# applied-geodesy/bundle-adjustment

Measured on AMD Instinct MI355X. Metric: LM iterations/sec, higher is better.
Workload: dtype f64

## Files before the change

### bundle-adjustment_amd/csrc/cholflow.hip

```cpp
#include <hip/hip_runtime.h>
#include <stdio.h>
#include <stdlib.h>
#include <string.h>

#include <algorithm>
#include <chrono>
#include <mutex>
#include <thread>
#include <vector>

#include "dense.h"
#include "gemm_f64.h"
#include "potrf_diag.h"

namespace jaicov {

#define HIPCHK(x)                                  \
    do {                                           \
        hipError_t _e = (x);                       \
        if (_e != hipSuccess) return _e;           \
    } while (0)

enum { FLOW_TICKET = 0, FLOW_ABORT = 1, FLOW_DIAG_NEXT = 2, FLOW_CHAIN_AT = 3, FLOW_STALE = 4, FLOW_STALE_CONFIRMED = 5, FLOW_RESCUED = 6, FLOW_WG_OFF = 7, FLOW_CTRL_WORDS = 16 };
constexpr int FLOW_FIN = 1 << 20;
constexpr int FLOW_PART = 1 << 21;
constexpr int FLOW_NPART_SHIFT = 22;
constexpr int FLOW_BUF_SHIFT = 12;
constexpr int FLOW_LDS = 144;
constexpr int FLOW_STAGE = GEMM_BK * 2 * FLOW_LDS;

struct FlowArgs {
    double *L;
    long ld;
    double *invd;
    const int4 *tasks;
    int n_tasks;
    int nb;
    int fs;
    int *ctrl;
    int *done;
    int *applied;
    int *diag_ready;
    int *factored;
    int *info;
    int *alive;
    int seq;
    const double *src;
    long src_ld;
    const double *V;
    const double *Bh;
    int d, U, bstride;
    double *diag_scratch;
    const double *zeros;
    double *scratch;
    double *partial;
    int *pflag;
    long long timeout;
    int fake_a;
    int crit_prio;
    int keep;
    int second_wg;
    int second_update;
    int inv_wt;
    int crit_span;
    int *wgstate;
    long long *ctrace;
    long long *trace;
};

__device__ __forceinline__ int flow_ld(const int *p) { return __hip_atomic_load(p, __ATOMIC_RELAXED, __HIP_MEMORY_SCOPE_AGENT); }
__device__ __forceinline__ int flow_ld_rmw(const int *p) { return __hip_atomic_fetch_or(const_cast<int *>(p), 0, __ATOMIC_RELAXED, __HIP_MEMORY_SCOPE_AGENT); }
__device__ __forceinline__ void flow_st(int *p, int v) { __hip_atomic_store(p, v, __ATOMIC_RELAXED, __HIP_MEMORY_SCOPE_SYSTEM); }
__device__ __forceinline__ int flow_ld_sys(const int *p) { return __hip_atomic_load(p, __ATOMIC_RELAXED, __HIP_MEMORY_SCOPE_SYSTEM); }
__device__ __forceinline__ void store_wt(double *p, double v) {
    __hip_atomic_store(reinterpret_cast<unsigned long long *>(p), (unsigned long long)__double_as_longlong(v), __ATOMIC_RELAXED,
                       __HIP_MEMORY_SCOPE_AGENT);
}
__device__ __forceinline__ void store_wt2(double *p, d2_t v) {
    asm volatile("s_nop 15\n\ts_nop 7\n\tglobal_store_dwordx4 %0, %1, off sc1\n\ts_nop 1" : : "v"(p), "v"(v) : "memory");
}
__device__ __forceinline__ void drain_stores() { asm volatile("s_waitcnt vmcnt(0)" ::: "memory"); }
#ifndef FLOW_LONG_NAP
#define FLOW_LONG_NAP 40
#endif

#define FLOW_OPAQUE_TID(name) int name = tid; asm volatile("" : "+v"(name))

__device__ __forceinline__ void flow_give_up(int *ctrl) {
    if (atomicCAS(ctrl + FLOW_ABORT, 0, 2) == 0) {
        int *wg = ctrl + ctrl[FLOW_WG_OFF];
        for (int b = 0; b < 1024; b++) wg[1024 + b] = flow_ld(wg + b);
    }
}

__device__ __forceinline__ bool flow_spin(const int *flag, int want, int *ctrl, long long timeout, long long *waited) {
    if (flow_ld(flag) >= want) return true;
    const long long t0 = wall_clock64();
    int spins = 0;
    bool ok = true;
    for (;;) {
        if (flow_ld(flag) >= want) break;
        if (++spins < 32) __builtin_amdgcn_s_sleep(4);
        else {
            __builtin_amdgcn_s_sleep(FLOW_LONG_NAP);
            if ((spins & 31) == 0) {
                if (flow_ld_sys(flag) >= want || flow_ld_rmw(flag) >= want) {
                    atomicAdd(ctrl + FLOW_STALE, 1);
                    if (flow_ld(flag) < want) atomicAdd(ctrl + FLOW_STALE_CONFIRMED, 1);
                    if (wall_clock64() - t0 > 100000) atomicAdd(ctrl + FLOW_RESCUED, 1);
                    break;
                }
                if (flow_ld(ctrl + FLOW_ABORT) != 0) { ok = false; break; }
                if (wall_clock64() - t0 > timeout) { flow_give_up(ctrl); ok = false; break; }
            }
        }
    }
    if (waited) *waited += wall_clock64() - t0;
    return ok;
}

__device__ __attribute__((noinline)) void flow_inline_diag(double *A, long ld, double *inv_out, int *info, int blk, double *ws) {
    potrf_diag_body(A, ld, inv_out, info, blk, 0, ws, ws + 128 * DP);
}

template <int PF, bool INLINE_DIAG>
__global__ __launch_bounds__(256, 2) void chol_tile_kernel(FlowArgs g) {
    __shared__ double smem[2 * FLOW_STAGE];
    __shared__ int s_msg[4];
    const int tid = threadIdx.x;
    const int bid = (int)blockIdx.x;

    d4_t acc[4][4];
    auto accumulate = [&](const double *Ap, long lda, const double *Bp, long ldb, int nk, double asign) __attribute__((always_inline)) {
        FLOW_OPAQUE_TID(tq);
        const int seg = tq & 7, rbase = tq >> 3, lane = tq & 63, wave = tq >> 6;
        const int odd = (seg & 1) * FLOW_LDS;
        const int st_lds = (2 * seg) * FLOW_LDS + rbase + 8 * ((seg >> 1) & 1) + 4 * (seg >> 2);
        const int fa = (lane >> 4) * FLOW_LDS + 64 * (wave >> 1) + (lane & 15);
        const int fb = (lane >> 4) * FLOW_LDS + 64 * (wave & 1) + (lane & 15);
        const double *ap = Ap + (long)rbase * lda + 2 * seg;
        const double *bp = Bp + (long)rbase * ldb + 2 * seg;
        d2_t ra[2][4], rb[2][4];
#define FLOW_GLOAD(S)                                                                                        \
    do {                                                                                                     \
        _Pragma("unroll") for (int q = 0; q < 4; q++) ra[S][q] = *reinterpret_cast<const d2_t *>(ap + (long)(32 * q) * lda); \
        _Pragma("unroll") for (int q = 0; q < 4; q++) rb[S][q] = *reinterpret_cast<const d2_t *>(bp + (long)(32 * q) * ldb); \
        ++ls;                                                                                                \
        const long adv = ls < nk ? GEMM_BK : 0;    \
        ap += adv;                                                                                           \
        bp += adv;                                                                                           \
    } while (0)
#define FLOW_LSTORE(S, STAGE)                                                                                \
    do {                                                                                                     \
        double *sa = smem + (STAGE) * FLOW_STAGE + st_lds;                                                   \
        double *sb = sa + GEMM_BK * FLOW_LDS;                                                                \
        _Pragma("unroll") for (int q = 0; q < 4; q++) {                                                      \
            sa[32 * q + odd] = asign * ra[S][q].x;                                                           \
            sa[32 * q + FLOW_LDS - odd] = asign * ra[S][q].y;                                                \
            sb[32 * q + odd] = rb[S][q].x;                                                                   \
            sb[32 * q + FLOW_LDS - odd] = rb[S][q].y;                                                        \
        }                                                                                                    \
    } while (0)
#define FLOW_FRAG(STAGE, KS, A_, B_)                                                                         \
    do {                                                                                                     \
        const double *sa = smem + (STAGE) * FLOW_STAGE + fa;                                                 \
        const double *sb = smem + (STAGE) * FLOW_STAGE + GEMM_BK * FLOW_LDS + fb;                            \
        const int sh = 8 * ((KS) & 1) + 4 * ((KS) >> 1);                                                     \
        _Pragma("unroll") for (int x = 0; x < 4; x++) A_[x] = sa[(4 * (KS)) * FLOW_LDS + 16 * x + sh];       \
        _Pragma("unroll") for (int y = 0; y < 4; y++) B_[y] = sb[(4 * (KS)) * FLOW_LDS + 16 * y + sh];       \
    } while (0)
#define FLOW_MM(A_, B_)                                                                                      \
    do {                                                                                                     \
        _Pragma("unroll") for (int x = 0; x < 4; x++)                                                        \
            _Pragma("unroll") for (int y = 0; y < 4; y++)                                                    \
                acc[x][y] = __builtin_amdgcn_mfma_f64_16x16x4f64(A_[x], B_[y], acc[x][y], 0, 0, 0);          \
    } while (0)
#define FLOW_MFMA(STAGE)                                                                                     \
    do {                                                                                                     \
        _Pragma("unroll") for (int ks = 0; ks < 4; ks++) {                                                   \
            double a[4], b[4];                                                                               \
            FLOW_FRAG(STAGE, ks, a, b);                                                                      \
            FLOW_MM(a, b);                                                                                   \
        }                                                                                                    \
    } while (0)
        int ls = 0;
        FLOW_GLOAD(0);
        if (PF == 2) {
            FLOW_GLOAD(1);
            FLOW_LSTORE(0, 0);
            __syncthreads();
            for (int kt = 0; kt < nk; kt += 2) {
                FLOW_GLOAD(0);
                FLOW_MFMA(0);
                FLOW_LSTORE(1, 1);
                __syncthreads();
                FLOW_GLOAD(1);
                FLOW_MFMA(1);
                FLOW_LSTORE(0, 0);
                __syncthreads();
            }
        } else {
            FLOW_LSTORE(0, 0);
            __syncthreads();
            for (int kt = 0; kt < nk; kt += 2) {
                FLOW_GLOAD(0);
                FLOW_MFMA(0);
                FLOW_LSTORE(0, 1);
                __syncthreads();
                FLOW_GLOAD(0);
                FLOW_MFMA(1);
                FLOW_LSTORE(0, 0);
                __syncthreads();
            }
        }
#undef FLOW_GLOAD
#undef FLOW_LSTORE
#undef FLOW_MFMA
#undef FLOW_FRAG
#undef FLOW_MM
    };

    if (!INLINE_DIAG && g.keep > 0 && (int)blockIdx.x >= g.keep) {
        const int xcc = 1 + (int)(__builtin_amdgcn_s_getreg((20 << 0) | (0 << 6) | (31 << 11)) & 0xf);
        if (xcc == flow_ld(g.ctrl + 9) || xcc == flow_ld(g.ctrl + 11) || (g.second_wg && xcc == flow_ld(g.ctrl + 13))) return;
    }
    for (;;) {
        if (tid == 0) s_msg[0] = atomicAdd(g.ctrl + FLOW_TICKET, 1);
        __syncthreads();
        const int t = s_msg[0];
        __syncthreads();
        if (t >= g.n_tasks) break;
        const int4 tk = g.tasks[t];
        const int ti = tk.x, tj = tk.y, k0 = tk.z & ((1 << FLOW_BUF_SHIFT) - 1), k1 = tk.w & (FLOW_FIN - 1);
        const int pbuf = tk.z >> FLOW_BUF_SHIFT, npart = (tk.w >> FLOW_NPART_SHIFT) & 7;
        const bool part = (tk.w & FLOW_PART) != 0;
        const bool first_visit = k0 == 0 || npart > 0;
#define FLOW_STAGE_MARK(kk, st) do { if (tid == 0) flow_st(g.wgstate + bid, (t << 12) | ((kk) << 4) | (st)); } while (0)
        FLOW_STAGE_MARK(k0, 1);
        const bool fin = (tk.w & FLOW_FIN) != 0;
        long long waited = 0, t_start = 0, t_c = 0, t_upd = 0, c_c = 0, c_upd = 0, w_upd = 0;
        int n_runs = 0;
        if (g.trace) t_start = wall_clock64();
        bool ok = true;
        const bool critical = ti <= tj + g.crit_span && g.crit_prio > 0;
        if (critical) __builtin_amdgcn_s_setprio(3);
        int k = k0;
        for (int phase = 0;; phase++) {
            if ((phase == 0 && !first_visit && !part) || phase == 1) {
                FLOW_STAGE_MARK(k, 2);
                if (tid == 0) {
                    const int *f = phase == 0 ? g.applied + (long)ti * g.fs + tj : g.done + (long)tj * g.fs + tj;
                    const bool r = flow_spin(f, phase == 0 ? k0 + 1 : 1, g.ctrl, g.timeout, &waited);
                    __builtin_amdgcn_fence(__ATOMIC_ACQUIRE, "agent");
                    drain_stores();
                    s_msg[1] = r ? 1 : 0;
                }
                __syncthreads();
                ok = s_msg[1] != 0;
                __syncthreads();
                if (!ok) break;
            }
            {
                FLOW_OPAQUE_TID(tq);
                const long trow = 64 * (tq >> 7) + ((tq & 63) >> 4), tcol = 64 * ((tq >> 6) & 1) + (tq & 15);
                const bool scaled = phase == 0 && first_visit && !part && g.src != nullptr && ti < g.nb;
                const double *src = phase != 0 || part ? g.zeros + (tq & 15)
                                    : scaled   ? g.src + ((long)ti * 128 + trow) * g.src_ld + (long)tj * 128 + tcol
                                               : g.L + ((long)ti * 128 + trow) * g.ld + (long)tj * 128 + tcol;
                const long sld = phase != 0 || part ? 0 : (scaled ? g.src_ld : g.ld);
#pragma unroll
                for (int x = 0; x < 4; x++)
#pragma unroll
                    for (int r = 0; r < 4; r++) {
                        const double *rowp = src + (long)(16 * x + 4 * r) * sld;
#pragma unroll
                        for (int y = 0; y < 4; y++) acc[x][y][r] = rowp[16 * y];
                    }
                if (scaled) {
                    const int R0 = ti * 128 + (int)trow, C0 = tj * 128 + (int)tcol;
                    double vc[4];
#pragma unroll
                    for (int y = 0; y < 4; y++) vc[y] = g.V[C0 + 16 * y];
#pragma unroll
                    for (int x = 0; x < 4; x++)
#pragma unroll
                        for (int r = 0; r < 4; r++) {
                            const int R = R0 + 16 * x + 4 * r;
                            const double vr = g.V[R];
#pragma unroll
                            for (int y = 0; y < 4; y++) {
                                const int Cc = C0 + 16 * y;
                                double v = vr * acc[x][y][r] * vc[y];
                                for (int a = 0; a < g.d; a++) v += g.Bh[(long)a * g.bstride + R] * g.Bh[(long)a * g.bstride + Cc];
                                const bool inside = R >= g.d && R < g.U && Cc >= g.d;
                                acc[x][y][r] = inside ? v : (R == Cc ? 1.0 : 0.0);
                            }
                        }
                }
            }
            if (g.trace && phase == 0) { t_c = wall_clock64(); c_c = clock64(); }
            for (bool more = true; more;) {
                const double *Ap, *Bp;
                long lda, ldb;
                int nk;
                double asign;
                if (phase == 0) {
                    if (k >= k1) break;
                    FLOW_STAGE_MARK(k, 3);
                    if (tid < 64) {
                        FLOW_OPAQUE_TID(lane);
                        const int *fi = g.done + (long)ti * g.fs, *fj = g.done + (long)tj * g.fs;
                        const long long t0 = wall_clock64();
                        int spins = 0, cnt = 0;
                        for (;;) {
                            const int idx = k + lane;
                            const bool ready = idx < k1 && flow_ld(fi + idx) != 0 && flow_ld(fj + idx) != 0;
                            const unsigned long long m = __ballot(ready);
                            cnt = m == ~0ull ? 64 : __builtin_ctzll(~m);
                            if (cnt > 0) break;
                            if (++spins < 32) __builtin_amdgcn_s_sleep(4);
                            else {
                                __builtin_amdgcn_s_sleep(FLOW_LONG_NAP);
                                if ((spins & 31) == 0) {
                                    if (wall_clock64() - t0 > 100000) {
                                        __builtin_amdgcn_fence(__ATOMIC_ACQUIRE, "agent");
                                        drain_stores();
                                    }
                                    const bool ready2 = idx < k1 && (flow_ld_sys(fi + idx) != 0 || flow_ld_rmw(fi + idx) != 0) &&
                                                        (flow_ld_sys(fj + idx) != 0 || flow_ld_rmw(fj + idx) != 0);
                                    const unsigned long long m2 = __ballot(ready2);
                                    cnt = m2 == ~0ull ? 64 : __builtin_ctzll(~m2);
                                    if (cnt > 0) {
                                        const bool again = idx < k1 && flow_ld(fi + idx) != 0 && flow_ld(fj + idx) != 0;
                                        const unsigned long long m3 = __ballot(again);
                                        if (lane == 0) {
                                            atomicAdd(g.ctrl + FLOW_STALE, 1);
                                            if ((m3 & 1ull) == 0) atomicAdd(g.ctrl + FLOW_STALE_CONFIRMED, 1);
                                            if (wall_clock64() - t0 > 100000) atomicAdd(g.ctrl + FLOW_RESCUED, 1);
                                        }
                                        break;
                                    }
                                    if (flow_ld(g.ctrl + FLOW_ABORT) != 0) break;
                                    if (wall_clock64() - t0 > g.timeout) { if (lane == 0) flow_give_up(g.ctrl); break; }
                                }
                            }
                        }
                        if (spins > 0) waited += wall_clock64() - t0;
                        __builtin_amdgcn_fence(__ATOMIC_ACQUIRE, "agent");
                        drain_stores();
                        if (lane == 0) {
                            s_msg[1] = cnt;
                            s_msg[2] = spins;
                        }
                    }
                    __syncthreads();
                    const int cnt = s_msg[1];
                    if (g.crit_prio >= 2 && s_msg[2] > 0) __builtin_amdgcn_s_setprio(3);
                    __syncthreads();
                    if (cnt == 0) { ok = false; break; }
                    ++n_runs;
                    FLOW_STAGE_MARK(k, 4);
                    Ap = g.L + (long)(g.fake_a ? tj : ti) * 128 * g.ld + (long)k * 128;
                    Bp = g.L + (long)tj * 128 * g.ld + (long)k * 128;
                    lda = ldb = g.ld;
                    nk = 8 * cnt;
                    asign = -1.0;
                    k += cnt;
                } else {
                    Ap = g.scratch + (long)bid * 16384;
                    Bp = g.invd + (long)tj * 16384;
                    lda = ldb = 128;
                    nk = 8;
                    asign = 1.0;
                    more = false;
                }
                accumulate(Ap, lda, Bp, ldb, nk, asign);
            }
            if (!ok) break;
            if (phase == 0 && npart > 0) {
                for (int q = 0; q < npart; q++) {
                    FLOW_STAGE_MARK(k, 9);
                    if (tid == 0) {
                        const bool r = flow_spin(g.pflag + pbuf + q, 1, g.ctrl, g.timeout, &waited);
                        __builtin_amdgcn_fence(__ATOMIC_ACQUIRE, "agent");
                        drain_stores();
                        s_msg[1] = r ? 1 : 0;
                    }
                    __syncthreads();
                    ok = s_msg[1] != 0;
                    __syncthreads();
                    if (!ok) break;
                    FLOW_OPAQUE_TID(tq);
                    const double *pp = g.partial + (long)(pbuf + q) * 16384 + (64 * (tq >> 7) + ((tq & 63) >> 4)) * 128 + 64 * ((tq >> 6) & 1) + (tq & 15);
#pragma unroll
                    for (int x = 0; x < 4; x++)
#pragma unroll
                        for (int r = 0; r < 4; r++)
#pragma unroll
                            for (int y = 0; y < 4; y++) acc[x][y][r] += pp[(16 * x + 4 * r) * 128 + 16 * y];
                }
                if (!ok) break;
            }
            if (g.trace && phase == 0) { t_upd = wall_clock64(); c_upd = clock64(); w_upd = waited; }
            FLOW_STAGE_MARK(k, 5 + phase);
            const bool to_scratch = phase == 0 && fin && ti != tj;
            {
                FLOW_OPAQUE_TID(tq);
                const long trow = 64 * (tq >> 7) + ((tq & 63) >> 4), tcol = 64 * ((tq >> 6) & 1) + (tq & 15);
                double *dst = part         ? g.partial + (long)pbuf * 16384 + trow * 128 + tcol
                              : to_scratch ? g.scratch + (long)bid * 16384 + trow * 128 + tcol
                                           : g.L + ((long)ti * 128 + trow) * g.ld + (long)tj * 128 + tcol;
                const long dld = part || to_scratch ? 128 : g.ld;
#pragma unroll
                for (int x = 0; x < 4; x++)
#pragma unroll
                    for (int r = 0; r < 4; r++) {
                        double *rowp = dst + (long)(16 * x + 4 * r) * dld;
#pragma unroll
                        for (int y = 0; y < 4; y++) store_wt(rowp + 16 * y, acc[x][y][r]);
                    }
            }
            drain_stores();
            if (to_scratch) continue;
            __syncthreads();
            if (INLINE_DIAG && phase == 0 && fin) {
                if (tid == 0) {
                    __builtin_amdgcn_fence(__ATOMIC_ACQUIRE, "agent");
                    drain_stores();
                }
                __syncthreads();
                double *ws = g.diag_scratch + (long)bid * (128 * DP + 8 * 16 * WDP);
                flow_inline_diag(g.L + (long)tj * 128 * g.ld + (long)tj * 128, g.ld, g.invd + (long)tj * 16384, g.info, tj, ws);
                drain_stores();
                __syncthreads();
                if (tid == 0) {
                    __builtin_amdgcn_fence(__ATOMIC_RELEASE, "agent");
                    drain_stores();
                    flow_st(g.done + (long)tj * g.fs + tj, 1);
                }
                break;
            }
            if (tid == 0) {
                if (part) flow_st(g.pflag + pbuf, 1);
                else if (phase == 1) flow_st(g.done + (long)ti * g.fs + tj, 1);
                else if (fin) flow_st(g.diag_ready + tj, 1);
                else flow_st(g.applied + (long)ti * g.fs + tj, k1 + 1);
            }
            break;
        }
        if (g.crit_prio > 0) __builtin_amdgcn_s_setprio(0);
        FLOW_STAGE_MARK(k, ok ? 7 : 8);
        if (!ok) break;
        if (g.trace && tid == 0) {
            long long *tr = g.trace + 8 * (long)t;
            tr[0] = t_start; tr[1] = t_c; tr[2] = t_upd; tr[3] = wall_clock64(); tr[4] = waited;
            tr[5] = c_upd - c_c;
            tr[6] = (long long)bid | ((long long)n_runs << 16) | (w_upd << 32);
            tr[7] = (long long)__builtin_amdgcn_s_getreg((4 << 0) | (0 << 6) | (31 << 11)) |
                    ((long long)(__builtin_amdgcn_s_getreg((20 << 0) | (0 << 6) | (31 << 11)) & 0xf) << 32);
// ... 797 lines not shown
```

### bundle-adjustment_amd/csrc/engine.hip

```cpp
#include <hip/hip_runtime.h>
#include <math.h>
#include <stdio.h>
#include <string.h>

#include <algorithm>
#include <atomic>
#include <chrono>
#include <string>
#include <vector>

#include "../../include/jaicov_dense.h"
#include "../../include/jaicov_neq.h"
#include "ba_kernels.h"
#include "batchinv.h"
#include "datum.h"
#include "dense.h"
#include "gemm_f64.h"
#include "reliability.h"
#include "transform.h"

namespace jaicov {
hipError_t launch_rows(hipStream_t, const DevProblem &, const double *, int, int, double *, double *);
hipError_t launch_assemble_small(hipStream_t, const DevProblem &, const int32_t *, const int32_t *, int, const double *,
                                 const double *, double, double *, double *);
hipError_t launch_assemble_blocks(hipStream_t, const DevProblem &, const int32_t *, int, int, const int32_t *, int,
                                  const double *, const double *, double *, double, double *, double *, const PPGather &,
                                  const SchurBufs &, double *, hipStream_t, hipEvent_t, hipEvent_t);
hipError_t launch_schur_backsub(hipStream_t, const DevProblem &, const int32_t *, int, const double *, const double *,
                                const double *, double *);
hipError_t launch_shared_groups(hipStream_t, const DevProblem &, const double *, double, double *, double *,
                                const double *, double *);
hipError_t launch_schur_expand_f(hipStream_t, const DevProblem &, const int32_t *, int, const double *, const double *, const double *,
                                 const double *, double *, long);
hipError_t launch_omega(hipStream_t, const DevProblem &, const uint8_t *, int, int, const int32_t *, int, int,
                        const double *, const double *, const double *, double, double *, double *);
struct RefineBorder { double kappa[7]; double rk[7]; };
hipError_t launch_residual_dd(hipStream_t, const double *, long, int, int, int, const double *, const double *, const double *,
                              const double *, const double *, long, const RefineBorder &, double *, double *);
}
using namespace jaicov;

static const double EPS53 = 1.1102230246251565e-16;

__global__ void damp_and_precond_kernel(double *N, long ld, int U, int Upad, int d, double lambda, double *V,
                                        const double *diagcorr) {
    const int c = blockIdx.x * blockDim.x + threadIdx.x;
    if (c >= Upad) return;
    double v = 1.0;
    if (c >= d && c < U) {
        double diag = N[(long)c * ld + c];
        if (lambda > 0.0) {
            diag += lambda * (diag + (diagcorr ? diagcorr[c] : 0.0));
            N[(long)c * ld + c] = diag;
        }
        v = diag > 1.1102230246251565e-16 ? 1.0 / sqrt(diag) : 1.0;
    }
    V[c] = v;
}

__global__ __launch_bounds__(256) void zero_lower_kernel(double *__restrict__ N, long ld, int rows, int skip_lo, int skip_hi, int row0) {
    const int r = row0 + blockIdx.y, c = 4 * (blockIdx.x * 256 + threadIdx.x);
    if (c > r || r >= rows) return;
    if (r >= skip_lo && r <= skip_hi) {
        if (c >= skip_lo) return;
        if (c + 4 > skip_lo) {
            for (int k = c; k < skip_lo; k++) N[(long)r * ld + k] = 0.0;
            return;
        }
    }
    *reinterpret_cast<d4_t *>(N + (long)r * ld + c) = (d4_t){0.0, 0.0, 0.0, 0.0};
}

__global__ __launch_bounds__(256) void scale_copy_kernel(const double *__restrict__ N, long ldN, double *__restrict__ M,
                                                         long ld, int U, int Upad, int d, const double *__restrict__ V,
                                                         const double *__restrict__ Bh, int bstride, int c_begin, int c_end) {
    const int j = c_begin + blockIdx.x * 256 + threadIdx.x;
    const int i = blockIdx.y;
    if (j > i || j >= c_end) return;
    double v;
    if (i < d || i >= U || j < d) v = (i == j) ? 1.0 : 0.0;
    else {
        v = V[i] * N[(long)i * ldN + j] * V[j];
        for (int a = 0; a < d; a++) v += Bh[(long)a * bstride + i] * Bh[(long)a * bstride + j];
    }
    M[(long)i * ld + j] = v;
}

__global__ void scale_vec_kernel(const double *n, const double *V, double *out, int U, int Upad, int d) {
    const int c = blockIdx.x * blockDim.x + threadIdx.x;
    if (c >= Upad) return;
    out[c] = (c >= d && c < U) ? V[c] * n[c] : 0.0;
}

__global__ __launch_bounds__(256) void qfix_kernel(double *__restrict__ Q, long ld, int U, int Upad, int d,
                                                   const double *__restrict__ V, const double *__restrict__ G, long gs,
                                                   const double *__restrict__ H, const double *__restrict__ F,
                                                   const double *__restrict__ E, int order) {
    const int j = blockIdx.x * 256 + threadIdx.x;
    const int i = blockIdx.y;
    if (j > i || j >= order) return;
    double v;
    if (i >= U) v = 0.0;
    else if (i < d) v = E[i * d + j];
    else if (j < d) v = F[(long)j * Upad + i];
    else {
        v = Q[(long)i * ld + j];
        for (int a = 0; a < d; a++) v -= G[(long)a * gs + i] * H[(long)a * Upad + j];
        v *= V[i] * V[j];
    }
    Q[(long)i * ld + j] = v;
}

__global__ __launch_bounds__(256) void expand_cofactor_kernel(double *__restrict__ Qf, long ldf, int U, int e0,
                                                              const double *__restrict__ Qr, long ldr,
                                                              const double *__restrict__ T1, long ld1,
                                                              const double *__restrict__ T2, long ld2,
                                                              const double *__restrict__ Linv) {
    const int j = blockIdx.x * 256 + threadIdx.x;
    const int i = blockIdx.y;
    if (j > i || i >= U) return;
    double v;
    if (i < e0) v = Qr[(long)i * ldr + j];
    else if (j < e0) v = T1[(long)(i - e0) * ld1 + j];
    else {
        const int ri = i - e0, rj = j - e0;
        v = T2[(long)ri * ld2 + rj];
        if (ri / 6 == rj / 6) {
            const double *Li = Linv + (long)(ri / 6) * 36;
            const int a = ri % 6, b = rj % 6;
            for (int m = a > b ? a : b; m < 6; m++) v += Li[6 * m + a] * Li[6 * m + b];
        }
    }
    Qf[(long)i * ldf + j] = v;
}

__global__ __launch_bounds__(256) void pack_kernel(const double *__restrict__ M, long ld, int U, double *__restrict__ ap) {
    const int j = blockIdx.x * 256 + threadIdx.x;
    const int i = blockIdx.y;
    if (j > i || i >= U) return;
    ap[(size_t)i * (i + 1) / 2 + j] = M[(long)i * ld + j];
}
__global__ __launch_bounds__(256) void unpack_kernel(const double *__restrict__ ap, long ld, int U, double *__restrict__ M) {
    const int j = blockIdx.x * 256 + threadIdx.x;
    const int i = blockIdx.y;
    if (j > i || i >= U) return;
    M[(long)i * ld + j] = ap[(size_t)i * (i + 1) / 2 + j];
}
__global__ void gather_sub_kernel(const double *__restrict__ Q, long ld, const int32_t *idx, int k, double *out, double scale) {
    const int t = blockIdx.x * blockDim.x + threadIdx.x;
    if (t >= k * k) return;
    const int a = t / k, b = t - a * k;
    const int i = idx[a], j = idx[b];
    out[t] = scale * (i >= j ? Q[(long)i * ld + j] : Q[(long)j * ld + i]);
}
__global__ void load_disp_kernel(const double *__restrict__ D, int m, double *__restrict__ L, long ld, int mp,
                                 const int32_t *__restrict__ perm) {
    const int j = blockIdx.x * 256 + threadIdx.x;
    const int i = blockIdx.y;
    if (j >= mp) return;
    double v = (i == j) ? 1.0 : 0.0;
    if (i < m && j < m) {
        const int si = perm ? 2 * perm[i >> 1] + (i & 1) : i, sj = perm ? 2 * perm[j >> 1] + (j & 1) : j;
        v = D[(long)si * m + sj];
    }
    L[(long)i * ld + j] = v;
}
__global__ void store_inv_kernel(const double *__restrict__ Q, long ld, int m, double *__restrict__ out) {
    const int j = blockIdx.x * 256 + threadIdx.x;
    const int i = blockIdx.y;
    if (j >= m) return;
    out[(long)i * m + j] = i >= j ? Q[(long)i * ld + j] : Q[(long)j * ld + i];
}

template <typename T>
// ... 1012 lines not shown
    if (inverse_follows == JAICOV_INVERT_NONE) return JAICOV_OK;
    HIPE(e, hipSetDevice(e->device));
    const bool reduced = e->schur_ok && (inverse_follows == JAICOV_INVERT_REDUCED || inverse_follows == JAICOV_INVERT_FULL_EXPANDED) && e->solverS_ready;
    return ensure_inverse_buffers(e, reduced, inverse_follows);
}

extern "C" int jaicov_neq_cofactor_order(const jaicov_engine *e) {
    if (!e || !e->have_Q) return -1;
    return e->q_order;
}

extern "C" int jaicov_neq_reduced_order(const jaicov_engine *e) {
    if (!e) return -1;
    return e->schur_active ? e->e0 : e->U;
}

extern "C" int jaicov_neq_accumulate2(jaicov_engine *e, double sigma2, double lambda) {
    if (!e) return JAICOV_ERR_BAD_ARGUMENT;
    e->lambda_acc = lambda > 0 ? lambda : 0.0;
    return jaicov_neq_accumulate(e, sigma2);
}

extern "C" int jaicov_neq_build(jaicov_engine *e, double sigma2, double lambda, int simulation) {
    if (!e) return JAICOV_ERR_BAD_ARGUMENT;
    e->lambda_acc = lambda > 0 ? lambda : 0.0;
    TRY(jaicov_neq_accumulate(e, sigma2));
    return jaicov_neq_finalize(e, sigma2, lambda, simulation);
}

static int reduce_buffer_impl(jaicov_engine *e, void **device_ptr, size_t *count, bool sync) {
    if (!e || !device_ptr || !count) return JAICOV_ERR_BAD_ARGUMENT;
    if (e->state != jaicov_engine::ST_ACCUMULATED) FAIL(e, JAICOV_ERR_BAD_STATE, "accumulate first");
    HIPE(e, hipSetDevice(e->device));
    const int Ua = e->schur_active ? e->e0 : e->U;
    const size_t len = (size_t)Ua * (Ua + 1) / 2;
    if (!e->d_packed) TRY(dalloc(e, (size_t)e->U * (e->U + 1) / 2 + 2 * (size_t)e->U, &e->d_packed));
    hipLaunchKernelGGL(pack_kernel, dim3((Ua + 255) / 256, std::max(Ua, 1)), dim3(256), 0, e->stream, e->d_N, (long)e->Upad, Ua, e->d_packed);
    HIPE(e, hipMemcpyAsync(e->d_packed + len, e->d_n, (size_t)Ua * sizeof(double), hipMemcpyDeviceToDevice, e->stream));
    if (e->schur_active)
        HIPE(e, hipMemcpyAsync(e->d_packed + len + Ua, e->sb.diagcorr, (size_t)Ua * sizeof(double), hipMemcpyDeviceToDevice, e->stream));
    if (sync) HIPE(e, hipStreamSynchronize(e->stream));
    e->reduced = true;
    *device_ptr = e->d_packed;
    *count = len + Ua + (e->schur_active ? (size_t)Ua : 0);
    return JAICOV_OK;
}

extern "C" int jaicov_neq_reduce_buffer(jaicov_engine *e, void **device_ptr, size_t *count) {
    return reduce_buffer_impl(e, device_ptr, count, true);
}

extern "C" int jaicov_neq_reduce_buffer_async(jaicov_engine *e, void **device_ptr, size_t *count, void **stream) {
    if (!stream) return JAICOV_ERR_BAD_ARGUMENT;
    const int rc = reduce_buffer_impl(e, device_ptr, count, false);
    if (rc == JAICOV_OK) *stream = (void *)e->stream;
    return rc;
}

static bool small_inverse(int d, const double *S, double *Sinv) {
    double a[7][14];
    for (int i = 0; i < d; i++)
        for (int j = 0; j < d; j++) { a[i][j] = S[i * d + j]; a[i][d + j] = i == j ? 1.0 : 0.0; }
    for (int c = 0; c < d; c++) {
        int piv = c;
        for (int r = c + 1; r < d; r++)
            if (fabs(a[r][c]) > fabs(a[piv][c])) piv = r;
        if (a[piv][c] == 0.0) return false;
        if (piv != c)
            for (int j = 0; j < 2 * d; j++) std::swap(a[c][j], a[piv][j]);
        const double inv = 1.0 / a[c][c];
        for (int j = 0; j < 2 * d; j++) a[c][j] *= inv;
        for (int r = 0; r < d; r++) {
            if (r == c) continue;
            const double f = a[r][c];
            if (f != 0.0)
                for (int j = 0; j < 2 * d; j++) a[r][j] -= f * a[c][j];
        }
    }
    for (int i = 0; i < d; i++)
        for (int j = 0; j < d; j++) Sinv[i * d + j] = a[i][d + j];
    return true;
}

struct Solve {
    jaicov_engine *const e;
    const bool schur;
    const int U, d, Upad;
    DenseSolver &slv;
    const int Up, vs;
    const long ld;
    int invert = 0;
    bool expand = false;
    std::vector<double> Bh, X, delta0;
    double R[7] = {1, 1, 1, 1, 1, 1, 1}, Sinv[49];
    bool fast_refined = false;
    float refine_ms = 0.f;
    explicit Solve(jaicov_engine *eng)
        : e(eng), schur(e->schur_active), U(schur ? e->e0 : e->U), d(e->d), Upad(e->Upad), slv(schur ? e->solverS : e->solver),
          Up(slv.nfact), vs(Up), ld(slv.ld) {}

    double border_dot(int a, const double *v) const {
        double s = 0.0;
        for (int c = d; c < U; c++) s += Bh[(size_t)a * Upad + c] * v[c];
        return s;
    }
    void border_multipliers(const double *v, const double *rk, double *k) const {
        double t[7];
        for (int a = 0; a < d; a++) t[a] = border_dot(a, v) - rk[a];
        for (int a = 0; a < d; a++) {
            double s = 0.0;
            for (int b = 0; b < d; b++) s += Sinv[a * d + b] * t[b];
            k[a] = s;
        }
    }

    int solve_mode(int requested) {
        invert = effective_invert(e, requested);
        if (invert == JAICOV_INVERT_FULL_EXPANDED && !schur) invert = JAICOV_INVERT_FULL;
        expand = invert == JAICOV_INVERT_FULL_EXPANDED;
        if (schur && invert == JAICOV_INVERT_FULL)
            FAIL(e, JAICOV_ERR_BAD_STATE, "the normal equations were assembled with the EO blocks pre-eliminated: call "
                                          "jaicov_neq_prepare_inverse(e, JAICOV_INVERT_FULL) before the build whose solve shall invert");
        slv.profile = e->solver.profile;
        slv.flops_order = (double)U;
        return invert ? ensure_inverse_buffers(e, schur, invert) : JAICOV_OK;
    }
    int border_rows() {
        int hinfo = 0;
        HIPE(e, hipMemcpyAsync(e->h_V.data(), e->d_V, Upad * sizeof(double), hipMemcpyDeviceToHost, e->stream));
        if (schur) HIPE(e, hipMemcpyAsync(&hinfo, e->sb.info, sizeof(int), hipMemcpyDeviceToHost, e->stream));
        HIPE(e, hipStreamSynchronize(e->stream));
        if (hinfo != 0) FAIL(e, JAICOV_ERR_SINGULAR, "exterior orientation block of image " + std::to_string(hinfo - 1000000) + " is not positive definite");
        Bh.assign((size_t)8 * Upad, 0.0);
        for (int a = 0; a < d; a++) {
            double s = 0.0;
            for (int c = d; c < U; c++) {
                const double v = e->hB[(size_t)a * Upad + c] * e->h_V[c];
                Bh[(size_t)a * Upad + c] = v;
                s += v * v;
            }
            if (!(s > 0.0)) FAIL(e, JAICOV_ERR_SINGULAR, "empty datum condition row");
            R[a] = 1.0 / sqrt(s);
            for (int c = d; c < U; c++) Bh[(size_t)a * Upad + c] *= R[a];
        }
        if (d > 0) HIPE(e, hipMemcpyAsync(e->d_B, Bh.data(), (size_t)d * Upad * sizeof(double), hipMemcpyHostToDevice, e->stream));
        HIPE(e, hipEventRecord(e->ev[4], e->stream));
        return JAICOV_OK;
    }
    int refine_begin() {
        const int nbk = Up / 128;
        HIPE(e, e->refP.reserve((size_t)nbk * nbk * 256));
        HIPE(e, hipEventRecord(e->ev_r0, e->stream));
        return JAICOV_OK;
    }
    int refine_step(const RefineBorder &bd, std::vector<double> &delta) {
        double *d_rhs = e->d_ref, *d_tmp = e->d_ref + Upad, *d_delta = e->d_ref + 2 * (size_t)Upad;
        HIPE(e, launch_residual_dd(e->stream, e->d_N, (long)Upad, U, d, Up, e->d_dx, e->d_n, e->d_V, e->d_Braw, e->d_B, (long)Upad,
                                   bd, e->refP.get(), d_rhs));
        HIPE(e, slv.solve_rhs(d_rhs, d_tmp, d_delta));
        HIPE(e, hipEventRecord(e->ev_r1, e->stream));
        delta.assign((size_t)Up, 0.0);
        HIPE(e, hipMemcpyAsync(delta.data(), d_delta, delta.size() * sizeof(double), hipMemcpyDeviceToHost, e->stream));
        return JAICOV_OK;
    }
    int apply_correction(const RefineBorder &bd, const std::vector<double> &dl, double *dx_out) {
        float ms1 = 0.f;
        hipEventElapsedTime(&ms1, e->ev_r0, e->ev_r1);
        refine_ms += ms1;
        double dk[7] = {0, 0, 0, 0, 0, 0, 0};
        border_multipliers(dl.data(), bd.rk, dk);
        double cmax = 0.0, xmax = 0.0;
        for (int c = d; c < U; c++) {
            double dy = dl[c];
            for (int a = 0; a < d; a++) dy -= X[(size_t)(1 + a) * vs + c] * dk[a];
            const double corr = e->h_V[c] * dy;
            if (!std::isfinite(corr)) FAIL(e, JAICOV_ERR_NOT_FINITE, "non-finite refinement step");
            dx_out[c] += corr;
            cmax = std::max(cmax, fabs(corr)); xmax = std::max(xmax, fabs(dx_out[c]));
        }
        for (int a = 0; a < d; a++) dx_out[a] += R[a] * dk[a];
        e->last_refine_correction = xmax > 0.0 ? cmax / xmax : 0.0;
        return JAICOV_OK;
    }
    int factor_and_substitute() {
        const int nrhs = d + 1;
        const bool fused = slv.flow_ready;
        const int c1 = std::min(slv.first_panel_cols(), Up);
        int info = 0;
        for (int attempt = 0;; attempt++) {
            HIPE(e, slv.begin_refactor());
            if (!fused)
                hipLaunchKernelGGL(scale_copy_kernel, dim3((c1 + 255) / 256, Up), dim3(256), 0, e->stream, e->d_N, (long)Upad, slv.L, ld, U,
                                   Up, d, e->d_V, e->d_B, Upad, 0, c1);
            HIPE(e, hipMemsetAsync(slv.rhs_row(0), 0, (size_t)128 * ld * sizeof(double), e->stream));
            hipLaunchKernelGGL(scale_vec_kernel, dim3((Up + 255) / 256), dim3(256), 0, e->stream, e->d_n, e->d_V, slv.rhs_row(0), U, Up, d);
            if (d > 0)
                HIPE(e, hipMemcpy2DAsync(slv.rhs_row(1), (size_t)ld * sizeof(double), e->d_B, (size_t)Upad * sizeof(double),
                                         (size_t)Up * sizeof(double), (size_t)d, hipMemcpyDeviceToDevice, e->stream));
            HIPE(e, hipEventRecord(e->ev_first, e->stream));
            if (!fused && c1 < Up)
                hipLaunchKernelGGL(scale_copy_kernel, dim3((Up - c1 + 255) / 256, Up), dim3(256), 0, e->stream, e->d_N, (long)Upad, slv.L,
                                   ld, U, Up, d, e->d_V, e->d_B, Upad, c1, Up);
            HIPE(e, hipEventRecord(e->ev_all, e->stream));
            if (fused) slv.flow_set_source(e->d_N, (long)Upad, e->d_V, e->d_B, Upad, d, U);
            HIPE(e, slv.potrf(e->ev_first, e->ev_all));
            HIPE(e, hipEventRecord(e->ev[5], e->stream));
            HIPE(e, slv.backsolve_aug(e->d_G, vs, nrhs));
            HIPE(e, hipEventRecord(e->ev[6], e->stream));
            X.assign((size_t)nrhs * vs, 0.0);
            HIPE(e, hipMemcpyAsync(X.data(), e->d_G, X.size() * sizeof(double), hipMemcpyDeviceToHost, e->stream));
            fast_refined = false;
            if (d == 0 && e->refine_steps >= 1 && !e->sim_built) {
                TRY(refine_begin());
                hipLaunchKernelGGL(scale_vec_kernel, dim3((Up + 255) / 256), dim3(256), 0, e->stream, e->d_G, e->d_V, e->d_dx, U, Up, 0);
                TRY(refine_step(RefineBorder{}, delta0));
                fast_refined = true;
            }
            info = slv.fetch_info();
            if (info == -9 && attempt < 2) {
                ++e->flow_retries;
                fprintf(stderr, "jaicov: factorisation abandoned on the device (a wait ran into its time limit); repeating it (%d)\n", attempt + 1);
                continue;
            }
            break;
        }
        if (info < 0) FAIL(e, JAICOV_ERR_DEVICE, "factorisation did not complete on the device (code " + std::to_string(info) + ")");
        if (info != 0) FAIL(e, JAICOV_ERR_SINGULAR, "normal-equation matrix is singular / not positive definite at pivot " + std::to_string(info));
        return JAICOV_OK;
    }
    int border_step(double *dx_out) {
        double Sm[49], kh[7];
        std::vector<double> y(X.begin(), X.begin() + vs);
        if (d > 0) {
            for (int a = 0; a < d; a++)
                for (int b = 0; b < d; b++) Sm[a * d + b] = border_dot(a, &X[(size_t)(1 + b) * vs]);
            if (!small_inverse(d, Sm, Sinv)) FAIL(e, JAICOV_ERR_SINGULAR, "datum conditions are linearly dependent");
            const double no_rk[7] = {0, 0, 0, 0, 0, 0, 0};
            border_multipliers(X.data(), no_rk, kh);
            for (int c = d; c < U; c++) {
                double s = 0.0;
                for (int a = 0; a < d; a++) s += X[(size_t)(1 + a) * vs + c] * kh[a];
                y[c] -= s;
            }
        }
        for (int c = 0; c < U; c++) dx_out[c] = c < d ? R[c] * kh[c] : e->h_V[c] * y[c];
        for (int c = 0; c < U; c++)
            if (!std::isfinite(dx_out[c])) FAIL(e, JAICOV_ERR_NOT_FINITE, "non-finite step");
        return JAICOV_OK;
    }
    int refine(double *dx_out) {
        e->last_refine_correction = 0.0;
        if (fast_refined) TRY(apply_correction(RefineBorder{}, delta0, dx_out));
        for (int step = fast_refined ? 1 : 0; step < e->refine_steps && !e->sim_built; step++) {
            RefineBorder bd{};
            for (int a = 0; a < d; a++) {
                long double sacc = 0.0L;
                for (int c = d; c < U; c++) sacc += (long double)e->hB[(size_t)a * Upad + c] * (long double)dx_out[c];
                bd.kappa[a] = dx_out[a];
                bd.rk[a] = (double)(-(long double)R[a] * sacc);
            }
            TRY(refine_begin());
            if (d > 0 && step == 0)
                HIPE(e, hipMemcpyAsync(e->d_Braw, e->hB.data(), (size_t)d * Upad * sizeof(double), hipMemcpyHostToDevice, e->stream));
            HIPE(e, hipMemcpyAsync(e->d_dx, dx_out, (size_t)U * sizeof(double), hipMemcpyHostToDevice, e->stream));
            std::vector<double> dl;
            TRY(refine_step(bd, dl));
            HIPE(e, hipStreamSynchronize(e->stream));
            TRY(apply_correction(bd, dl, dx_out));
        }
        return JAICOV_OK;
    }
    int eo_backsub() {
        HIPE(e, launch_omega(e->stream, e->p, e->d_in_block, e->ip0, e->ip_count, e->d_blk_list, 0, e->max_m, e->d_rowsA,
                             e->d_rowsW, e->d_dx, 1.0, e->d_vbuf, e->d_omega));
        HIPE(e, launch_schur_backsub(e->stream, e->p, e->d_blk_list, e->n_blk_list, e->sb.U, e->sb.Linv, e->d_vbuf, e->d_xE));
        return JAICOV_OK;
    }
    int eo_zero_step_guard(std::vector<double> &xE) {
        bool all_zero = !e->h_blk_images.empty();
        for (int img : e->h_blk_images)
            for (int k = 0; k < 6 && all_zero; k++) all_zero = xE[(size_t)6 * img + k] == 0.0;
        if (!all_zero) return JAICOV_OK;
        HIPE(e, hipDeviceSynchronize());
        HIPE(e, hipMemcpy(xE.data(), e->d_xE, xE.size() * sizeof(double), hipMemcpyDeviceToHost));
        bool still = true;
        for (int img : e->h_blk_images)
            for (int k = 0; k < 6 && still; k++) still = xE[(size_t)6 * img + k] == 0.0;
        if (still) {
            TRY(eo_backsub());
            HIPE(e, hipStreamSynchronize(e->stream));
            HIPE(e, hipMemcpy(xE.data(), e->d_xE, xE.size() * sizeof(double), hipMemcpyDeviceToHost));
        }
        fprintf(stderr, "jaicov: the exterior-orientation step came back as exact zeros; %s\n",
                still ? "the back-substitution was run again" : "a second, blocking copy had the values (the first copy returned before the data)");
        return JAICOV_OK;
    }
    int eo_entries(double *dx_out) {
        const bool quirk = e->opts.reduced_reference_quirk && invert == JAICOV_INVERT_REDUCED;
        if (schur)
            for (int c = U; c < e->U; c++) dx_out[c] = 0.0;
        if (schur && e->sim_built) return JAICOV_OK;
        if (schur && quirk) {
            std::vector<double> xq((size_t)6 * e->p.n_images);
            HIPE(e, hipMemcpyAsync(xq.data(), e->sb.xq, xq.size() * sizeof(double), hipMemcpyDeviceToHost, e->stream));
            HIPE(e, hipStreamSynchronize(e->stream));
            for (int img : e->h_blk_images)
                for (int k = 0; k < 6; k++) dx_out[e->e0 + 6 * img + k] = xq[(size_t)6 * img + k];
        } else if (schur) {
            HIPE(e, hipMemcpyAsync(e->d_dx, dx_out, (size_t)e->U * sizeof(double), hipMemcpyHostToDevice, e->stream));
            TRY(eo_backsub());
            std::vector<double> xE((size_t)6 * e->p.n_images);
            HIPE(e, hipMemcpyAsync(xE.data(), e->d_xE, xE.size() * sizeof(double), hipMemcpyDeviceToHost, e->stream));
            HIPE(e, hipStreamSynchronize(e->stream));
            TRY(eo_zero_step_guard(xE));
            for (int img : e->h_blk_images)
                for (int k = 0; k < 6; k++) {
                    dx_out[e->e0 + 6 * img + k] = xE[(size_t)6 * img + k];
                    if (!std::isfinite(xE[(size_t)6 * img + k])) FAIL(e, JAICOV_ERR_NOT_FINITE, "non-finite step");
                }
        } else if (quirk) {
            std::vector<double> hn((size_t)e->U);
            HIPE(e, hipMemcpyAsync(hn.data(), e->d_n, hn.size() * sizeof(double), hipMemcpyDeviceToHost, e->stream));
            HIPE(e, hipStreamSynchronize(e->stream));
            const int ns = e->n_slots, s_eo = ns - 6 * e->p.n_images;
            for (int sl = s_eo; sl < ns; sl++) {
                const int c = e->h_slot_col[sl];
                if (c >= 0) dx_out[c] = e->h_V[c] * e->h_V[c] * hn[c];
            }
        }
        return JAICOV_OK;
    }
    int invert_and_expand() {
        HIPE(e, slv.trtri());
        HIPE(e, slv.lauum());
        if (e->opts.inverse_refinement >= 0 && Up <= 8192) {
            const size_t sq = (size_t)Up * ld;
            HIPE(e, e->ns_work.reserve(3 * sq));
            double *ns = e->ns_work.get();
            HIPE(e, slv.begin_refactor());
            HIPE(e, slv.symmetrize(slv.Q));
            hipLaunchKernelGGL(scale_copy_kernel, dim3((Up + 255) / 256, Up), dim3(256), 0, e->stream, e->d_N, (long)Upad, slv.L, ld, U,
                               Up, d, e->d_V, e->d_B, Upad, 0, Up);
            HIPE(e, slv.symmetrize(slv.L));
            HIPE(e, newton_schulz_exact(e->stream, Up, ld, slv.L, slv.Q, slv.W, ns, ns + sq, ns + 2 * sq));
        }
        std::vector<double> H((size_t)8 * Upad, 0.0), F((size_t)8 * Upad, 0.0);
        double E[49];
        for (int a = 0; a < d; a++) {
            for (int c = d; c < U; c++) {
                double s = 0.0;
                for (int b = 0; b < d; b++) s += Sinv[a * d + b] * X[(size_t)(1 + b) * vs + c];
                H[(size_t)a * Upad + c] = s;
                F[(size_t)a * Upad + c] = R[a] * s * e->h_V[c];
            }
            for (int b = 0; b < d; b++) E[a * d + b] = R[a] * ((a == b ? 1.0 : 0.0) - Sinv[a * d + b]) * R[b];
        }
        if (d > 0) {
            HIPE(e, hipMemcpyAsync(e->d_H, H.data(), (size_t)d * Upad * sizeof(double), hipMemcpyHostToDevice, e->stream));
            HIPE(e, hipMemcpyAsync(e->d_F, F.data(), (size_t)d * Upad * sizeof(double), hipMemcpyHostToDevice, e->stream));
            HIPE(e, hipMemcpyAsync(e->d_E, E, (size_t)d * d * sizeof(double), hipMemcpyHostToDevice, e->stream));
        }
        hipLaunchKernelGGL(qfix_kernel, dim3((Up + 255) / 256, Up), dim3(256), 0, e->stream, slv.Q, ld, U, Upad, d,
                           e->d_V, e->d_G + vs, (long)vs, e->d_H, e->d_F, e->d_E, Up);
        return expand ? expand_cofactor() : JAICOV_OK;
    }
    int expand_cofactor() {
        size_t I6, UpS;
        if (!expansion_fits(e, &I6, &UpS))
            FAIL(e, JAICOV_ERR_UNSUPPORTED, "FULL_EXPANDED: more exterior orientations than the workspace holds; use JAICOV_INVERT_FULL");
        const int I6p = (int)I6;
        double *Fm = slv.W, *T1 = Fm + (size_t)I6p * Up, *T2 = T1 + (size_t)I6p * Up;
        const double *LinvAll = e->sb.Linv;
        if (e->all_images) {
            HIPE(e, hipMemsetAsync(Fm, 0, (size_t)I6p * Up * sizeof(double), e->stream));
            HIPE(e, launch_schur_expand_f(e->stream, e->p, e->d_blk_list, e->n_blk_list, e->d_rowsA, e->sb.U, e->sb.Linv, e->sb.G, Fm, (long)Up));
        } else {
            if (!e->exp_ready || e->expF_len != (size_t)I6p * Up + (size_t)36 * e->p.n_images)
                FAIL(e, JAICOV_ERR_BAD_STATE, "FULL_EXPANDED on a sharded engine: all-reduce jaicov_neq_expansion_buffer() between accumulate and solve");
            HIPE(e, hipMemcpyAsync(Fm, e->expF.get(), (size_t)I6p * Up * sizeof(double), hipMemcpyDeviceToDevice, e->stream));
            LinvAll = e->expF.get() + (size_t)I6p * Up;
        }
        HIPE(e, slv.symmetrize(slv.Q));
        GemmArgs g1{};
        g1.A = Fm; g1.lda = Up; g1.B = slv.Q; g1.ldb = ld; g1.C = T1; g1.ldc = Up;
        g1.M = I6p; g1.N = Up; g1.K = Up; g1.alpha = -1.0; g1.beta = 0.0; g1.kmode = KMODE_FULL;
        HIPE(e, gemm_f64(e->stream, LAY_KC, LAY_KC, g1));
        GemmArgs g2{};
        g2.A = T1; g2.lda = Up; g2.B = Fm; g2.ldb = Up; g2.C = T2; g2.ldc = I6p;
        g2.M = I6p; g2.N = I6p; g2.K = Up; g2.alpha = -1.0; g2.beta = 0.0; g2.kmode = KMODE_FULL; g2.lower_only = 1;
        HIPE(e, gemm_f64(e->stream, LAY_KC, LAY_KC, g2));
        hipLaunchKernelGGL(expand_cofactor_kernel, dim3((e->U + 255) / 256, e->U), dim3(256), 0, e->stream, e->solver.Q, e->solver.ld,
                           e->U, e->e0, slv.Q, ld, T1, (long)Up, T2, (long)I6p, LinvAll);
        return JAICOV_OK;
    }
    int finish() {
        HIPE(e, hipEventRecord(e->ev[7], e->stream));
// ... 620 lines not shown
```

Before: 38.65.

## Keep the exterior-orientation back-substitution on device and trim RHS tile MFMAs

In the Schur path with one refinement step, the refined correction is now added to dx on the device and the exterior-orientation back-substitution runs immediately. This removes a host round trip: copy X and delta to the host, rebuild dx there, then copy it back before eo_backsub. Separately, Cholesky tiles whose row index equals nb (the right-hand-side block row) now issue only the MFMAs needed for 16 rows, and the second half of the workgroup issues none. The risks are divergence from the host-computed dx, since the add is done with explicit rn ops, and reliance on an env var and a debug counter.

```diff
diff --git a/bundle-adjustment_amd/csrc/cholflow.hip b/bundle-adjustment_amd/csrc/cholflow.hip
--- a/bundle-adjustment_amd/csrc/cholflow.hip
+++ b/bundle-adjustment_amd/csrc/cholflow.hip
@@ -26,6 +26,7 @@
 constexpr int FLOW_PART = 1 << 21;
 constexpr int FLOW_NPART_SHIFT = 22;
 constexpr int FLOW_BUF_SHIFT = 12;
+constexpr int FLOW_RHS_ROWS = 16;
 constexpr int FLOW_LDS = 144;
 constexpr int FLOW_STAGE = GEMM_BK * 2 * FLOW_LDS;
 
@@ -131,7 +132,7 @@
     const int bid = (int)blockIdx.x;
 
     d4_t acc[4][4];
-    auto accumulate = [&](const double *Ap, long lda, const double *Bp, long ldb, int nk, double asign) __attribute__((always_inline)) {
+    auto accumulate = [&](const double *Ap, long lda, const double *Bp, long ldb, int nk, double asign, int xlim) __attribute__((always_inline)) {
         FLOW_OPAQUE_TID(tq);
         const int seg = tq & 7, rbase = tq >> 3, lane = tq & 63, wave = tq >> 6;
         const int odd = (seg & 1) * FLOW_LDS;
@@ -172,8 +173,9 @@
 #define FLOW_MM(A_, B_)                                                                                      \
     do {                                                                                                     \
         _Pragma("unroll") for (int x = 0; x < 4; x++)                                                        \
-            _Pragma("unroll") for (int y = 0; y < 4; y++)                                                    \
-                acc[x][y] = __builtin_amdgcn_mfma_f64_16x16x4f64(A_[x], B_[y], acc[x][y], 0, 0, 0);          \
+            if (x < xlim)                                                                                    \
+                _Pragma("unroll") for (int y = 0; y < 4; y++)                                                \
+                    acc[x][y] = __builtin_amdgcn_mfma_f64_16x16x4f64(A_[x], B_[y], acc[x][y], 0, 0, 0);      \
     } while (0)
 #define FLOW_MFMA(STAGE)                                                                                     \
     do {                                                                                                     \
@@ -243,6 +245,11 @@
         if (g.trace) t_start = wall_clock64();
         bool ok = true;
         const bool critical = ti <= tj + g.crit_span && g.crit_prio > 0;
+        int xlim;
+        {
+            FLOW_OPAQUE_TID(tw);
+            xlim = __builtin_amdgcn_readfirstlane(ti == g.nb ? ((tw >> 7) == 0 ? FLOW_RHS_ROWS / 16 : 0) : 4);
+        }
         if (critical) __builtin_amdgcn_s_setprio(3);
         int k = k0;
         for (int phase = 0;; phase++) {
@@ -374,7 +381,7 @@
                     asign = 1.0;
                     more = false;
                 }
-                accumulate(Ap, lda, Bp, ldb, nk, asign);
+                accumulate(Ap, lda, Bp, ldb, nk, asign, xlim);
             }
             if (!ok) break;
             if (phase == 0 && npart > 0) {
diff --git a/bundle-adjustment_amd/csrc/engine.hip b/bundle-adjustment_amd/csrc/engine.hip
--- a/bundle-adjustment_amd/csrc/engine.hip
+++ b/bundle-adjustment_amd/csrc/engine.hip
@@ -90,6 +90,12 @@
     const int c = blockIdx.x * blockDim.x + threadIdx.x;
     if (c >= Upad) return;
     out[c] = (c >= d && c < U) ? V[c] * n[c] : 0.0;
+}
+
+__global__ void add_scaled_kernel(const double *delta, const double *V, double *dx, int U, int Uall) {
+    const int c = blockIdx.x * blockDim.x + threadIdx.x;
+    if (c >= Uall) return;
+    dx[c] = c < U ? __dadd_rn(dx[c], __dmul_rn(V[c], delta[c])) : 0.0;
 }
 
 __global__ __launch_bounds__(256) void qfix_kernel(double *__restrict__ Q, long ld, int U, int Upad, int d,
@@ -1268,6 +1274,9 @@
     return true;
 }
 
+static std::atomic<long> g_device_tails{0};
+extern "C" long jaicov_debug_device_tails() { return g_device_tails.load(); }
+
 struct Solve {
     jaicov_engine *const e;
     const bool schur;
@@ -1280,6 +1289,8 @@
     std::vector<double> Bh, X, delta0;
     double R[7] = {1, 1, 1, 1, 1, 1, 1}, Sinv[49];
     bool fast_refined = false;
+    bool eo_on_device = false;
+    std::vector<double> xE;
     float refine_ms = 0.f;
     explicit Solve(jaicov_engine *eng)
         : e(eng), schur(e->schur_active), U(schur ? e->e0 : e->U), d(e->d), Upad(e->Upad), slv(schur ? e->solverS : e->solver),
@@ -1339,15 +1350,23 @@
         HIPE(e, hipEventRecord(e->ev_r0, e->stream));
         return JAICOV_OK;
     }
-    int refine_step(const RefineBorder &bd, std::vector<double> &delta) {
+    int refine_step(const RefineBorder &bd, std::vector<double> &delta, bool copy_out = true) {
         double *d_rhs = e->d_ref, *d_tmp = e->d_ref + Upad, *d_delta = e->d_ref + 2 * (size_t)Upad;
         HIPE(e, launch_residual_dd(e->stream, e->d_N, (long)Upad, U, d, Up, e->d_dx, e->d_n, e->d_V, e->d_Braw, e->d_B, (long)Upad,
                                    bd, e->refP.get(), d_rhs));
         HIPE(e, slv.solve_rhs(d_rhs, d_tmp, d_delta));
         HIPE(e, hipEventRecord(e->ev_r1, e->stream));
         delta.assign((size_t)Up, 0.0);
-        HIPE(e, hipMemcpyAsync(delta.data(), d_delta, delta.size() * sizeof(double), hipMemcpyDeviceToHost, e->stream));
+        if (copy_out) HIPE(e, fetch_delta(delta));
         return JAICOV_OK;
+    }
+    hipError_t fetch_delta(std::vector<double> &delta) {
+        return hipMemcpyAsync(delta.data(), e->d_ref + 2 * (size_t)Upad, delta.size() * sizeof(double), hipMemcpyDeviceToHost, e->stream);
+    }
+    bool tail_on_device() const {
+        const bool quirk = e->opts.reduced_reference_quirk && invert == JAICOV_INVERT_REDUCED;
+        const char *env = getenv("JAICOV_SOLVE_TAIL");
+        return schur && e->all_images && e->refine_steps == 1 && !quirk && !(env && !strcmp(env, "host"));
     }
     int apply_correction(const RefineBorder &bd, const std::vector<double> &dl, double *dx_out) {
         float ms1 = 0.f;
@@ -1394,14 +1413,25 @@
             HIPE(e, slv.backsolve_aug(e->d_G, vs, nrhs));
             HIPE(e, hipEventRecord(e->ev[6], e->stream));
             X.assign((size_t)nrhs * vs, 0.0);
-            HIPE(e, hipMemcpyAsync(X.data(), e->d_G, X.size() * sizeof(double), hipMemcpyDeviceToHost, e->stream));
-            fast_refined = false;
+            fast_refined = eo_on_device = false;
             if (d == 0 && e->refine_steps >= 1 && !e->sim_built) {
+                eo_on_device = tail_on_device();
+                if (!eo_on_device) HIPE(e, hipMemcpyAsync(X.data(), e->d_G, X.size() * sizeof(double), hipMemcpyDeviceToHost, e->stream));
                 TRY(refine_begin());
                 hipLaunchKernelGGL(scale_vec_kernel, dim3((Up + 255) / 256), dim3(256), 0, e->stream, e->d_G, e->d_V, e->d_dx, U, Up, 0);
-                TRY(refine_step(RefineBorder{}, delta0));
+                TRY(refine_step(RefineBorder{}, delta0, !eo_on_device));
                 fast_refined = true;
-            }
+                if (eo_on_device) {
+                    hipLaunchKernelGGL(add_scaled_kernel, dim3((e->U + 255) / 256), dim3(256), 0, e->stream, e->d_ref + 2 * (size_t)Upad, e->d_V,
+                                       e->d_dx, U, e->U);
+                    TRY(eo_backsub());
+                    HIPE(e, hipMemcpyAsync(X.data(), e->d_G, X.size() * sizeof(double), hipMemcpyDeviceToHost, e->stream));
+                    HIPE(e, fetch_delta(delta0));
+                    xE.assign((size_t)6 * e->p.n_images, 0.0);
+                    HIPE(e, hipMemcpyAsync(xE.data(), e->d_xE, xE.size() * sizeof(double), hipMemcpyDeviceToHost, e->stream));
+                }
+            } else
+                HIPE(e, hipMemcpyAsync(X.data(), e->d_G, X.size() * sizeof(double), hipMemcpyDeviceToHost, e->stream));
             info = slv.fetch_info();
             if (info == -9 && attempt < 2) {
                 ++e->flow_retries;
@@ -1412,6 +1442,7 @@
         }
         if (info < 0) FAIL(e, JAICOV_ERR_DEVICE, "factorisation did not complete on the device (code " + std::to_string(info) + ")");
         if (info != 0) FAIL(e, JAICOV_ERR_SINGULAR, "normal-equation matrix is singular / not positive definite at pivot " + std::to_string(info));
+        if (eo_on_device) ++g_device_tails;
         return JAICOV_OK;
     }
     int border_step(double *dx_out) {
@@ -1493,11 +1524,13 @@
             for (int img : e->h_blk_images)
                 for (int k = 0; k < 6; k++) dx_out[e->e0 + 6 * img + k] = xq[(size_t)6 * img + k];
         } else if (schur) {
-            HIPE(e, hipMemcpyAsync(e->d_dx, dx_out, (size_t)e->U * sizeof(double), hipMemcpyHostToDevice, e->stream));
-            TRY(eo_backsub());
-            std::vector<double> xE((size_t)6 * e->p.n_images);
-            HIPE(e, hipMemcpyAsync(xE.data(), e->d_xE, xE.size() * sizeof(double), hipMemcpyDeviceToHost, e->stream));
-            HIPE(e, hipStreamSynchronize(e->stream));
+            if (!eo_on_device) {
+                HIPE(e, hipMemcpyAsync(e->d_dx, dx_out, (size_t)e->U * sizeof(double), hipMemcpyHostToDevice, e->stream));
+                TRY(eo_backsub());
+                xE.assign((size_t)6 * e->p.n_images, 0.0);
+                HIPE(e, hipMemcpyAsync(xE.data(), e->d_xE, xE.size() * sizeof(double), hipMemcpyDeviceToHost, e->stream));
+                HIPE(e, hipStreamSynchronize(e->stream));
+            }
             TRY(eo_zero_step_guard(xE));
             for (int img : e->h_blk_images)
                 for (int k = 0; k < 6; k++) {
```

Result: no change. 38.37, median of 2 (-0.7%).
